# cebarker1000/heatflow

Measured on AMD Instinct MI355X. Metric: DOF-updates/s (timesteps/s x nDOF) on geballe_with_diamond, higher is better.
Workload: dtype f64

## Files before the change

heatflow_amd/csrc/heatflow_hip.hip:

```cpp

#include "hf_amg_io.hpp"

namespace {

struct MeshTables {
  std::vector<int32_t> rowptr, colidx;
  ColDict spmv;
  RowGather rg;
  std::vector<char> tag_used;
  int max_blk_nnz = 0;
};

constexpr char BLOB_MAGIC[8] = {'H', 'F', 'P', 'A', 'T', '0', '2', 0};
struct BlobHeader {
  char magic[8];
  int64_t total_bytes, nnz;
  int32_t n, ne, rba, ts, max_blk_nnz, tab_len, rg_ok, rg_max_dict, spmv_max_dict, reserved;
  int64_t count[12];
};

void steady_swap(hf_ctx* ctx) {
  hf_ctx::Steady& S = ctx->steady;
  std::swap(ctx->nbc, S.nbc); std::swap(ctx->d_bc_dofs, S.bc_dofs); std::swap(ctx->d_g, S.g);
  std::swap(ctx->nlift_rows, S.nlift_rows); std::swap(ctx->nlift, S.nlift);
  std::swap(ctx->d_lift_rows, S.lift_rows); std::swap(ctx->d_lift_ptr, S.lift_ptr); std::swap(ctx->d_lift_bc, S.lift_bc);
  std::swap(ctx->d_lift_slot, S.lift_slot); std::swap(ctx->d_lift_val, S.lift_val);
  std::swap(ctx->d_A, S.K); std::swap(ctx->d_dinv, S.dinv);
  std::swap(ctx->amg, S.amg); std::swap(ctx->d_coarse_inv, S.coarse_inv); std::swap(ctx->d_coarse_inv_f, S.coarse_inv_f);
  std::swap(ctx->coarse_n, S.coarse_n); std::swap(ctx->coarse_ld, S.coarse_ld); std::swap(ctx->amg_ready, S.amg_ready);
  std::swap(ctx->amg_fine_stale, S.amg_fine_stale); std::swap(ctx->amg_opc, S.amg_opc); std::swap(ctx->amg_setup_s, S.amg_setup_s);
  std::swap(ctx->amg_print, S.amg_print);
}
struct SteadyScope {
  hf_ctx* c;
  explicit SteadyScope(hf_ctx* ctx) : c(ctx) { steady_swap(c); }
  ~SteadyScope() { steady_swap(c); }
  SteadyScope(const SteadyScope&) = delete;
  SteadyScope& operator=(const SteadyScope&) = delete;
};

void steady_free(hf_ctx* ctx) {
  {
    SteadyScope sw(ctx);
    free_amg(ctx);
  }
  hf_ctx::Steady& S = ctx->steady;
  dev_free(&S.bc_dofs); dev_free(&S.g); dev_free(&S.lift_rows); dev_free(&S.lift_ptr); dev_free(&S.lift_bc);
  dev_free(&S.lift_slot); dev_free(&S.lift_val); dev_free(&S.K); dev_free(&S.dinv); dev_free(&S.Kfree);
  S.nbc = S.nlift_rows = S.nlift = 0;
  S.ready = false;
  S.pred_iters = 0;
}

void load_free(hf_ctx* ctx) {
  dev_free(&ctx->d_load);
  ctx->have_load = false;
}

void tangent_free(hf_ctx* ctx) {
  free_batch_state(ctx->tanb);
  dev_free(&ctx->tan.col); dev_free(&ctx->tan.F);
  ctx->tan = hf_ctx::Tangent();
}
// ... 17 lines not shown
  ctx->max_chunk_nnz_s = 0;
  for (int c = 0; c < ctx->nchunks_s; ++c)
    ctx->max_chunk_nnz_s = std::max(ctx->max_chunk_nnz_s, T.rowptr[std::min<int64_t>(n, (c + 1LL) * SRPC)] - T.rowptr[static_cast<size_t>(c) * SRPC]);
  ctx->max_cdict = T.spmv.max_dict;
  ctx->c16 = true;
  if (const char* e = std::getenv("HEATFLOW_SPMV_C16")) ctx->c16 = (e[0] != '0');
  if (static_cast<size_t>(ctx->max_chunk_nnz_s + ctx->max_cdict) * 8 > 64 * 1024) ctx->c16 = false;
  ctx->cdict_own = static_cast<int>(T.spmv.ptr.size()) == ctx->nchunks_s + 1;
  for (int c = 0; c < ctx->nchunks_s && ctx->cdict_own; ++c) {
    const int32_t r0 = c * SRPC, r1 = std::min<int32_t>(n, r0 + SRPC);
    const int32_t* lo = T.spmv.dict.data() + T.spmv.ptr[c];
    const int32_t* hi = T.spmv.dict.data() + T.spmv.ptr[c + 1];
    const int32_t* at = std::lower_bound(lo, hi, r0);
    ctx->cdict_own = hi - at >= r1 - r0 && at[0] == r0 && at[r1 - r0 - 1] == r1 - 1;
  }
  ctx->max_blk_nnz = T.max_blk_nnz;
  if (static_cast<size_t>((ctx->max_blk_nnz + 1) & ~1) * 16 + (RBA + 1) * 4 > 160 * 1024)
    return fail(ctx, HF_ERR_ARG, "row block holds %d nonzeros: LDS slab too large", ctx->max_blk_nnz);
  ctx->tab_len = static_cast<int>(T.tag_used.size());
  ctx->h_tag_used = T.tag_used;
  ctx->assembled = false; ctx->have_mat = false;
  ctx->h_tri.assign(tri, tri + 3 * static_cast<size_t>(ne));
  ctx->h_tag.assign(tag, tag + ne);
  ctx->owner_ready = false;
  ctx->ncolors = 0; ctx->elist_len = 0;
  dev_free(&ctx->d_blk_eptr); dev_free(&ctx->d_blk_cptr); dev_free(&ctx->d_blk_ent);

  std::vector<int4> elem(ne);
  for (int32_t e = 0; e < ne; ++e) elem[e] = make_int4(tri[3 * e], tri[3 * e + 1], tri[3 * e + 2], tag[e]);
  HF_TRY(dev_alloc(ctx, &ctx->d_zr, n));
// ... 442 lines not shown
  *out = ctx;
  return rc;
}

int hf_destroy(hf_ctx* ctx) {
  if (!ctx) return HF_ERR_ARG;
  (void)hipSetDevice(ctx->dev);
  if (ctx->stream) (void)hipStreamSynchronize(ctx->stream);
  dev_free(&ctx->d_zr); dev_free(&ctx->d_elem); dev_free(&ctx->d_kappa); dev_free(&ctx->d_rhoc);
  dev_free(&ctx->d_rowptr); dev_free(&ctx->d_colidx); dev_free(&ctx->d_cdict_ptr); dev_free(&ctx->d_cdict); dev_free(&ctx->d_cid); dev_free(&ctx->d_blk_eptr); dev_free(&ctx->d_blk_cptr); dev_free(&ctx->d_blk_ent); dev_free(&ctx->d_rg_hdr); dev_free(&ctx->d_rg_ell); dev_free(&ctx->d_rg_cid); dev_free(&ctx->d_rg_dict); dev_free(&ctx->d_rg_zrb); dev_free(&ctx->d_kappa_rg); dev_free(&ctx->d_rhoc_rg); dev_free(&ctx->d_M); dev_free(&ctx->d_A); dev_free(&ctx->d_dinv);
  dev_free(&ctx->d_bc_dofs); dev_free(&ctx->d_g); dev_free(&ctx->d_lift_rows); dev_free(&ctx->d_lift_ptr);
  dev_free(&ctx->d_lift_bc); dev_free(&ctx->d_lift_slot); dev_free(&ctx->d_lift_val);
  dev_free(&ctx->d_uprev); dev_free(&ctx->d_ustart);
  dev_free(&ctx->d_u); dev_free(&ctx->d_b); dev_free(&ctx->d_r); dev_free(&ctx->d_p); dev_free(&ctx->d_Ap);
  free_batch(ctx); free_batch_state(ctx->fluxb); free_batch_cols(ctx); free_amg(ctx); free_responses(ctx); proj_free(ctx); dev_free(&ctx->d_z); dev_free(&ctx->d_z2);
  steady_free(ctx); load_free(ctx); tangent_free(ctx);
  dev_free(&ctx->d_M1); dev_free(&ctx->d_dinv1); dev_free(&ctx->d_gz); dev_free(&ctx->d_gr); dev_free(&ctx->d_bz); dev_free(&ctx->d_br);
  dev_free(&ctx->d_tmp); dev_free(&ctx->d_part_pAp); dev_free(&ctx->d_part_rz); dev_free(&ctx->d_part_zz);
  dev_free(&ctx->d_part_bn); dev_free(&ctx->d_scal); dev_free(&ctx->d_samp_idx); dev_free(&ctx->d_samp); dev_free(&ctx->d_fsamp_idx);
  for (auto& e : ctx->prof_ev) (void)hipEventDestroy(e);
  if (ctx->h_scal) (void)hipHostFree(ctx->h_scal);
  if (ctx->h_mirror) (void)hipHostFree(ctx->h_mirror);
  if (ctx->ev0) (void)hipEventDestroy(ctx->ev0);
  if (ctx->ev1) (void)hipEventDestroy(ctx->ev1);
  if (ctx->stream) (void)hipStreamDestroy(ctx->stream);
  delete ctx;
  return HF_OK;
}

int hf_set_mesh(hf_ctx* ctx, int32_t n, int32_t ne, const double* zr, const int32_t* tri, const int32_t* tag) {
  if (!ctx) return HF_ERR_ARG;
// ... 138 lines not shown
  ctx->dt = ctx->scheme == HF_TIME_BDF2 ? 2.0 * dt / 3.0 : dt;
  ctx->mode = mode;
  HF_HIP(hipEventRecord(ctx->ev0, ctx->stream));
  HF_TRY(launch_assemble(ctx));
  if (ctx->nbc > 0) {
    if (ctx->nlift > 0)
      hipLaunchKernelGGL(k_take_lift, dim3((ctx->nlift + 255) / 256), dim3(256), 0, ctx->stream, ctx->nlift,
                         ctx->d_lift_slot, ctx->d_A, ctx->d_lift_val);
    hipLaunchKernelGGL(k_bc_rows, dim3((ctx->nbc + 255) / 256), dim3(256), 0, ctx->stream, ctx->nbc, ctx->d_bc_dofs,
                       ctx->d_rowptr, ctx->d_colidx, ctx->d_A);
  }
  hipLaunchKernelGGL(k_dinv, dim3((ctx->n + 255) / 256), dim3(256), 0, ctx->stream, ctx->n, ctx->d_rowptr,
                     ctx->d_colidx, ctx->d_A, ctx->d_dinv);
  HF_HIP(hipEventRecord(ctx->ev1, ctx->stream));
  HF_HIP(hipGetLastError());
  HF_HIP(hipStreamSynchronize(ctx->stream));
  float ms = 0.f;
  HF_HIP(hipEventElapsedTime(&ms, ctx->ev0, ctx->ev1));
  ctx->last_ms = ms;
  if (ctx->precond == 1) {
    OperatorPrint now;
    HF_TRY(operator_print(ctx, now));
    if (!(ctx->amg_ready && ctx->amg_reuse)) {
      HF_TRY(build_amg_auto(ctx));
      ctx->amg_print = std::move(now);
    } else {
      ctx->amg_fine_stale = !same_print(now, ctx->amg_print);
    }
  }
  if (ctx->precond == 1 && ctx->amg_ready) {
    ctx->amg[0].A.val = ctx->d_A;
// ... 492 lines not shown
  HF_HIP(copy_sync(ctx, S.bc_dofs, dofs, sizeof(int32_t) * n_s, hipMemcpyHostToDevice));
  HF_HIP(hipEventRecord(ctx->ev0, ctx->stream));
  HF_TRY(launch_assemble_rows<true>(ctx, ctx->d_kappa_rg, ctx->d_rhoc_rg, 1.0, nullptr, S.Kfree));
  HF_HIP(hipMemcpyAsync(S.K, S.Kfree, sizeof(double) * ctx->nnz, hipMemcpyDeviceToDevice, ctx->stream));
  {
    SteadyScope sw(ctx);
    HF_TRY(build_lift(ctx));
    if (ctx->nlift > 0)
      hipLaunchKernelGGL(k_take_lift, dim3((ctx->nlift + 255) / 256), dim3(256), 0, ctx->stream, ctx->nlift, ctx->d_lift_slot,
                         ctx->d_A, ctx->d_lift_val);
    hipLaunchKernelGGL(k_bc_rows, dim3((ctx->nbc + 255) / 256), dim3(256), 0, ctx->stream, ctx->nbc, ctx->d_bc_dofs, ctx->d_rowptr,
                       ctx->d_colidx, ctx->d_A);
    hipLaunchKernelGGL(k_dinv, dim3((n + 255) / 256), dim3(256), 0, ctx->stream, n, ctx->d_rowptr, ctx->d_colidx, ctx->d_A, ctx->d_dinv);
    HF_HIP(hipEventRecord(ctx->ev1, ctx->stream));
    HF_HIP(hipGetLastError());
    HF_HIP(hipStreamSynchronize(ctx->stream));
    float ms = 0.f;
    HF_HIP(hipEventElapsedTime(&ms, ctx->ev0, ctx->ev1));
    ctx->last_ms = ms;
    if (precond == 1) HF_TRY(build_amg_auto(ctx));
  }
  S.precond = precond;
  S.pred_iters = 0;
  S.ready = true;
  return HF_OK;
}

int hf_steady_solve(hf_ctx* ctx, const double* g_s, int32_t use_load, double rtol, double atol, int32_t max_it, int32_t* iters,
                    double* resid) {
  if (!ctx) return HF_ERR_ARG;
  if (!ctx->steady.ready) return fail(ctx, HF_ERR_STATE, "hf_steady_solve before hf_steady_setup (or the materials changed since)");
// ... 433 lines not shown
```

heatflow_amd/csrc/hf_context.hpp:

```cpp

#pragma once
#include <hip/hip_runtime.h>
#include <hip/hip_ext.h>

#include <algorithm>
#include <chrono>
#include <cmath>
#include <cstdarg>
#include <cstdint>
#include <cstdio>
#include <cstdlib>
#include <cstring>
#include <string>
#include <thread>
#include <vector>

#include "amg_host.hpp"
#include "heatflow_hip.h"

namespace {

constexpr int RB = 256;
#ifndef HF_RBA
#define HF_RBA 256
// ... 60 lines not shown
  hipStream_t stream = nullptr;
  hipEvent_t ev0 = nullptr, ev1 = nullptr;
  std::string err;
  double last_ms = 0.0;

  int32_t n = 0, ne = 0, nbc = 0;
  int64_t nnz = 0;
  int nchunks = 0, P = 0;
  int nchunks_s = 0, Ps = 0;
  int max_chunk_nnz_s = 0;
  int32_t *d_cdict_ptr = nullptr, *d_cdict = nullptr;
  uint16_t* d_cid = nullptr;
  int max_cdict = 0;
  bool cdict_own = false;
  bool c16 = true;
  bool have_mesh = false, have_mat = false, assembled = false;
  double dt = 0.0;
  double dt_step = 0.0;
  int mode = 0;
  int scheme = HF_TIME_BACKWARD_EULER;

  std::vector<int32_t> h_rowptr, h_colidx, h_tri, h_tag;
  std::vector<char> h_tag_used;
  bool owner_ready = false;

  double2* d_zr = nullptr;
  int4* d_elem = nullptr;
  int tab_len = 0;
  double *d_kappa = nullptr, *d_rhoc = nullptr;
  int32_t *d_rowptr = nullptr, *d_colidx = nullptr;
// ... 64 lines not shown
    double *dinv = nullptr, *x = nullptr, *cat = nullptr, *b = nullptr, *res = nullptr;
    bool own_b = false;
    double omega = 0; int n = 0;
  };
  std::vector<DevLevel> amg;
  double* d_coarse_inv = nullptr;
  float* d_coarse_inv_f = nullptr;
  int coarse_n = 0, coarse_ld = 0;
  bool amg_fine_stale = false;
  int amg_fuse0 = 0;
  bool amg_f32 = true;
  double amg_opc = 0.0, amg_setup_s = 0.0;
  struct OperatorPrint { double dt = 0.0; std::vector<double> kappa, rhoc; int32_t nbc = 0; uint64_t bc_hash = 0; int32_t scheme = 0; } amg_print;
  long long amg_fallbacks = 0;
  struct Steady {
    bool ready = false;
    int precond = 0, pred_iters = 0;
    int32_t nbc = 0, nlift_rows = 0, nlift = 0;
    int32_t *bc_dofs = nullptr, *lift_rows = nullptr, *lift_ptr = nullptr, *lift_bc = nullptr, *lift_slot = nullptr;
    double *g = nullptr, *lift_val = nullptr, *K = nullptr, *dinv = nullptr, *Kfree = nullptr;
    std::vector<DevLevel> amg;
    double* coarse_inv = nullptr;
    float* coarse_inv_f = nullptr;
    int coarse_n = 0, coarse_ld = 0;
    bool amg_ready = false, amg_fine_stale = false;
    double amg_opc = 0.0, amg_setup_s = 0.0;
    OperatorPrint amg_print;
  } steady;
  double* d_load = nullptr;
  bool have_load = false;
// ... 121 lines not shown
```

heatflow_amd/csrc/hf_kernels.hpp:

```cpp
#pragma once
#include "hf_context.hpp"

namespace {


template <int NW = 4>
__device__ __forceinline__ double block_sum(double v, double* sw) {
#pragma unroll
  for (int o = 32; o > 0; o >>= 1) v += __shfl_down(v, o, 64);
  const int w = threadIdx.x >> 6;
  if ((threadIdx.x & 63) == 0) sw[w] = v;
  __syncthreads();
  double t = sw[0];
#pragma unroll
  for (int k = 1; k < NW; ++k) t += sw[k];
  __syncthreads();
  return t;
}

__device__ __forceinline__ double sum_partials(const double* __restrict__ part, int P, double* s4) {
  double v = 0.0;
  for (int k = threadIdx.x; k < P; k += TPB) v += part[k];
  return block_sum(v, s4);
}
// ... 507 lines not shown
  const int q = blockIdx.x * blockDim.x + threadIdx.x;
  if (q < ns) out[q] = u[idx[q]];
}

__global__ __launch_bounds__(TPB) void k_hold_load(int n, const int32_t* __restrict__ rowptr, const int32_t* __restrict__ colidx,
                                                   const double* __restrict__ K, const double* __restrict__ u,
                                                   const unsigned char* __restrict__ mask, double* __restrict__ F) {
  const int row = blockIdx.x * blockDim.x + threadIdx.x;
  if (row >= n) return;
  double s = 0.0;
  if (!mask[row])
    for (int k = rowptr[row]; k < rowptr[row + 1]; ++k) s += K[k] * u[colidx[k]];
  F[row] = s;
}

__global__ void k_mark_rows(int nq, const int32_t* __restrict__ idx, unsigned char* __restrict__ mask) {
  const int q = blockIdx.x * blockDim.x + threadIdx.x;
  if (q < nq) mask[idx[q]] = 1;
}

__device__ __forceinline__ unsigned long long mirror_stamp(unsigned epoch, int v) {
  return (static_cast<unsigned long long>(epoch) << 32) | static_cast<unsigned>(v);
}
__device__ __forceinline__ void mirror_publish(ScalMirror* m, double zz, int iters, int done, unsigned epoch) {
  if (m == nullptr) return;
  m->zz = zz;
  m->iters = iters;
  __hip_atomic_store(&m->done_st, mirror_stamp(epoch, done), __ATOMIC_RELAXED, __HIP_MEMORY_SCOPE_SYSTEM);
  __threadfence_system();
  __hip_atomic_store(&m->tested_st, mirror_stamp(epoch, iters + 1), __ATOMIC_RELEASE, __HIP_MEMORY_SCOPE_SYSTEM);
}
__device__ __forceinline__ void mirror_breakdown(ScalMirror* m, unsigned epoch) {
  if (m != nullptr) __hip_atomic_store(&m->done_st, mirror_stamp(epoch, 2), __ATOMIC_RELEASE, __HIP_MEMORY_SCOPE_SYSTEM);
}

struct ColComp { const int32_t* dptr; const int32_t* dict; const uint16_t* id; int xd_off; int own; };

#ifndef HF_NT_STREAM
#define HF_NT_STREAM 0
#endif
#ifndef HF_PIPE
#define HF_PIPE 1
#endif
#ifndef HF_PHASE_CLOCK
#define HF_PHASE_CLOCK -1
#endif
#if HF_PHASE_CLOCK >= 0
#ifndef HF_PHASE_CONV
#define HF_PHASE_CONV 0
#endif
__device__ unsigned long long g_phase[MAXP * 16];
// ... 2 lines not shown
    if (MODE == HF_PHASE_CLOCK && C16 && (MODE != 0 || (part2 != nullptr) == (HF_PHASE_CONV != 0)) && threadIdx.x == 0 && (slot) < 16) \
      g_phase[blockIdx.x * 16 + (slot)] = wall_clock64();                                                \
  } while (0)
#else
#define HF_STAMP(slot) do { } while (0)
#endif
template <typename T>
__device__ __forceinline__ T stream_load(const T* p) {
#if HF_NT_STREAM
  return __builtin_nontemporal_load(p);
#else
  return *p;
#endif
}

__device__ __forceinline__ double bdf2_operand(double un, double unm1) { return (4.0 * un - unm1) * (1.0 / 3.0); }

template <int MODE, bool C16 = false, typename VT = double, int UN = 8>
__global__ __launch_bounds__(TS) __attribute__((amdgpu_waves_per_eu(8, 8))) void k_spmv(int n, int nchunks, int rpc ,
                                              const int32_t* __restrict__ rowptr, const int32_t* __restrict__ colidx,
                                              const VT* __restrict__ vals, const double* __restrict__ x,
                                              double* __restrict__ y, Scal* __restrict__ scal,
                                              double* __restrict__ part0, const double* __restrict__ bvec,
                                              const double* __restrict__ dinv, double* __restrict__ pvec,
                                              double* __restrict__ part1, double* __restrict__ part2, double w,
                                              int npart ,
                                              int parity, ColComp comp) {
  extern __shared__ double sprod[];
  __shared__ double s4[TS / 64];
  __shared__ int s_own;
  constexpr bool BDF = MODE >= 12 && MODE <= 15;
  auto opnd = [&](int c) { return BDF ? bdf2_operand(x[c], bvec[c]) : x[c]; };
  if ((MODE == 3 || MODE == 4 || MODE == 6 || MODE == 9) && scal->done) return;
  if ((MODE == 0 || MODE == 7) && scal != nullptr && scal->done) return;
  double acc0 = 0.0, acc1 = 0.0, acc2 = 0.0;
  double beta = 0.0;
  bool first9 = false;
  if (MODE == 9) {
    first9 = scal->first != 0;
    if (!first9) {
      double v0 = 0.0, v1 = 0.0, v2 = 0.0;
      for (int k = threadIdx.x; k < npart; k += TS) {
        v0 += part1[parity * MAXP + k];
        v1 += part1[(parity ^ 1) * MAXP + k];
        v2 += part2[k];
// ... 10 lines not shown
      beta = rz_new / rz_old;
    }
  }
  auto cycle_gate = [&]() {
    if (!((MODE == 3 || MODE == 0) && part2 != nullptr)) return false;
    double v2 = 0.0;
    for (int k = threadIdx.x; k < npart; k += TS) v2 += part2[k];
    const double zz = block_sum<TS / 64>(v2, s4);
    const bool conv = zz <= scal->tol2;
    if (blockIdx.x == 0 && threadIdx.x == 0) {
      if (conv) { scal->zz = zz; scal->done = 1; }
      mirror_publish(scal->mirror, zz, scal->iters, conv ? 1 : 0, scal->epoch);
    }
    return conv;
  };
  constexpr bool PIPELINED = C16 && (HF_PIPE == 2 || (HF_PIPE == 1 && sizeof(VT) == 4));
  if (!PIPELINED && cycle_gate()) return;
  const ChunkIter sched(nchunks);
  HF_STAMP(0);
  int stamp_at = 1;
  (void)stamp_at;
  const int tpr = (MODE == 0 || MODE == 6 || MODE == 7) ? TS / rpc : 1;
  const int prel = static_cast<int>(threadIdx.x) / tpr;
  const int psub = static_cast<int>(threadIdx.x) % tpr;
  struct RowOps { double b, d, y, p, x; };
  auto row_operands = [&](int prc, bool from_slice) {
    RowOps e{0.0, 0.0, 0.0, 0.0, 0.0};
    if (MODE == 2 || MODE == 3 || MODE == 4 || MODE == 5 || MODE == 7 || MODE == 8 || MODE == 11 || MODE == 13 || MODE == 15) e.b = bvec[prc];
    if (MODE == 2 || MODE == 4 || MODE == 5 || MODE == 10 || MODE == 11 || MODE == 14 || MODE == 15) e.d = dinv[prc];
    if (MODE == 6 || (MODE == 9 && !first9)) e.y = y[prc];
    if (MODE == 9 && !first9) e.p = pvec[prc];
    if ((MODE == 4 || MODE == 8 || MODE == 9 || MODE == 11) && !from_slice) e.x = x[prc];
    if (BDF) e.x = x[prc];
    return e;
  };
  auto rows_phase = [&](bool pin, int prow, int pa, int pb, const RowOps& e) {
    if ((MODE == 0 || MODE == 6 || MODE == 7) && tpr > 1) {
      double s = 0.0;
      if (pin)
        for (int j = pa + psub; j < pb; j += tpr) s += sprod[j];
      for (int o = tpr >> 1; o > 0; o >>= 1) s += __shfl_down(s, o, 64);
      if (pin && psub == 0) {
        y[prow] = (MODE == 6) ? e.y + s : s;
        if (MODE == 7) acc0 += e.b * s;
      }
    } else if (pin) {
      const int row = prow;
      double s = 0.0;
      for (int j = pa; j < pb; ++j) s += sprod[j];
      if (MODE == 0) {
        y[row] = s;
      } else if (MODE == 2) {
        const double ri = e.b - s;
        const double zi = e.d * ri;
        y[row] = ri;
        pvec[row] = zi;
        acc0 += ri * zi;
        acc1 += zi * zi;
        acc2 += (e.d * e.b) * (e.d * e.b);
      } else if (MODE == 3) {
        y[row] = e.b - s;
      } else if (MODE == 4) {
        const double yi = e.x + w * e.d * (e.b - s);
        y[row] = yi;
// ... 125 lines not shown
    }
  } else {
  const ChunkIter& sched_ = sched;
  for (int chunk = sched_.chunk; chunk < sched_.end; chunk += sched_.step) {
    const int r0 = chunk * rpc;
    const int r1 = min(n, r0 + rpc);
    const int k0 = rowptr[r0];
    const int k1 = rowptr[r1];
    const int prow = r0 + prel;
    const bool pin = prow < r1;
    int pa = 0, pb = 0;
    if (pin) {
      pa = rowptr[prow] - k0;
      pb = rowptr[prow + 1] - k0;
    }
    RowOps e = row_operands(min(prow, r1 - 1), C16 && comp.own != 0);
    if (C16) {
      double* xd = sprod + comp.xd_off;
      const int d0 = comp.dptr[chunk], nd = comp.dptr[chunk + 1] - d0;
      int k = k0 + threadIdx.x;
      double v[HF_UNROLL];
      int id[HF_UNROLL];
#pragma unroll
      for (int u = 0; u < HF_UNROLL; ++u) {
        const bool in = k + u * TS < k1;
        v[u] = in ? static_cast<double>(stream_load(&vals[k + u * TS])) : 0.0;
        id[u] = in ? static_cast<int>(stream_load(&comp.id[k + u * TS])) : 0;
      }
      for (int i = threadIdx.x; i < nd; i += HF_STAGE_U * TS) {
        int c[HF_STAGE_U];
        double xv[HF_STAGE_U];
#pragma unroll
        for (int u = 0; u < HF_STAGE_U; ++u) c[u] = (i + u * TS < nd) ? comp.dict[d0 + i + u * TS] : 0;
#pragma unroll
        for (int u = 0; u < HF_STAGE_U; ++u) xv[u] = (i + u * TS < nd) ? opnd(c[u]) : 0.0;
#pragma unroll
        for (int u = 0; u < HF_STAGE_U; ++u)
          if (i + u * TS < nd) {
            xd[i + u * TS] = xv[u];
            if ((MODE == 4 || MODE == 8 || MODE == 9 || MODE == 11) && c[u] == r0) s_own = i + u * TS;
          }
      }
      __syncthreads();
      HF_STAMP(stamp_at); ++stamp_at;
      if ((MODE == 4 || MODE == 8 || MODE == 9 || MODE == 11) && comp.own && pin) e.x = xd[s_own + (prow - r0)];
      while (k < k1) {
        const int kn = k + HF_UNROLL * TS;
        double vn[HF_UNROLL];
        int idn[HF_UNROLL];
#pragma unroll
        for (int u = 0; u < HF_UNROLL; ++u) {
          const bool in = kn + u * TS < k1;
          vn[u] = in ? static_cast<double>(stream_load(&vals[kn + u * TS])) : 0.0;
          idn[u] = in ? static_cast<int>(stream_load(&comp.id[kn + u * TS])) : 0;
        }
#pragma unroll
        for (int u = 0; u < HF_UNROLL; ++u)
          if (k + u * TS < k1) sprod[k - k0 + u * TS] = v[u] * xd[id[u]];
#pragma unroll
        for (int u = 0; u < HF_UNROLL; ++u) { v[u] = vn[u]; id[u] = idn[u]; }
        k = kn;
      }
    } else {
      for (int k = k0 + threadIdx.x; k < k1; k += HF_UNROLL * TS) {
        int c[HF_UNROLL];
        double v[HF_UNROLL], xv[HF_UNROLL];
#pragma unroll
        for (int u = 0; u < HF_UNROLL; ++u) {
          const bool in = k + u * TS < k1;
          c[u] = in ? colidx[k + u * TS] : 0;
          v[u] = in ? static_cast<double>(vals[k + u * TS]) : 0.0;
        }
#pragma unroll
        for (int u = 0; u < HF_UNROLL; ++u) xv[u] = (k + u * TS < k1) ? opnd(c[u]) : 0.0;
#pragma unroll
        for (int u = 0; u < HF_UNROLL; ++u)
          if (k + u * TS < k1) sprod[k - k0 + u * TS] = v[u] * xv[u];
      }
    }
    __syncthreads();
    HF_STAMP(stamp_at); ++stamp_at;
    rows_phase(pin, prow, pa, pb, e);
    __syncthreads();
    HF_STAMP(stamp_at); ++stamp_at;
  }
  }
  if (MODE == 2 || MODE == 7 || MODE == 9 || (MODE == 4 && part0 != nullptr)) {
    const double t0 = block_sum<TS / 64>(acc0, s4);
    if (threadIdx.x == 0) {
      part0[blockIdx.x] = t0;
      for (int q = blockIdx.x + gridDim.x; q < npart; q += gridDim.x) part0[q] = 0.0;
    }
  }
  if (MODE == 2 || MODE == 5) {
    const double t1 = block_sum<TS / 64>(acc1, s4);
    const double t2 = block_sum<TS / 64>(acc2, s4);
    if (threadIdx.x == 0) {
// ... 534 lines not shown
```

heatflow_amd/csrc/hf_pattern.hpp:

```cpp
#pragma once
#include <thread>

#include "hf_kernels.hpp"

namespace {

struct ColDict {
  std::vector<int32_t> ptr, dict;
  std::vector<uint16_t> id;
  int max_dict = 0;
};

struct RowGather {
  bool ok = false;
  std::vector<int4> hdr;
  std::vector<uint16_t> ell;
  std::vector<int32_t> tags;
  ColDict cols;
};

struct OwnerLists {
  std::vector<int32_t> blk_eptr, blk_cptr, blk_elist;
  std::vector<int2> blk_ent;
  int ncolors = 0;
// ... 331 lines not shown
  if (ctx->mode == HF_ASM_ROW_GATHER)
    return launch_assemble_lds(ctx, true, ctx->d_kappa, ctx->d_rhoc, ctx->dt, ctx->d_M, ctx->d_A);
  if (ctx->mode == HF_ASM_LDS_COLORED || ctx->mode == HF_ASM_LDS_ATOMIC) {
    return launch_assemble_lds(ctx, ctx->mode == HF_ASM_LDS_COLORED, ctx->d_kappa, ctx->d_rhoc, ctx->dt, ctx->d_M, ctx->d_A);
  } else {
    HF_HIP(hipMemsetAsync(ctx->d_M, 0, sizeof(double) * ctx->nnz, ctx->stream));
    HF_HIP(hipMemsetAsync(ctx->d_A, 0, sizeof(double) * ctx->nnz, ctx->stream));
    hipLaunchKernelGGL(k_assemble_global, dim3((ctx->ne + TPB - 1) / TPB), dim3(TPB), 0, ctx->stream, ctx->ne,
                       ctx->d_rowptr, ctx->d_colidx, ctx->d_elem, ctx->d_zr, ctx->d_kappa, ctx->d_rhoc, ctx->dt,
                       ctx->d_M, ctx->d_A);
  }
  HF_HIP(hipGetLastError());
  return HF_OK;
}

template <int MODE, typename VT = double>
void launch_spmv(hf_ctx* c, const VT* vals, const double* x, double* y, double* part0 = nullptr,
                 const double* bvec = nullptr, double* pvec = nullptr, double* part1 = nullptr,
                 double* part2 = nullptr, double w = 0.0, const double* dinv = nullptr, hipEvent_t ev_start = nullptr,
                 hipEvent_t ev_stop = nullptr, int parity = 0) {
  const ColComp comp{c->d_cdict_ptr, c->d_cdict, c->d_cid, c->max_chunk_nnz_s, c->cdict_own ? 1 : 0};
#define HF_SPMV_ARGS c->n, c->nchunks_s, static_cast<int>(SRPC), static_cast<const int32_t*>(c->d_rowptr),                    \
                     static_cast<const int32_t*>(c->d_colidx), vals, x, y, (MODE == 0 ? nullptr : c->d_scal), part0, bvec,  \
                     dinv ? dinv : static_cast<const double*>(c->d_dinv), pvec, part1, part2, w, c->P, parity, comp
  const std::uint32_t smem = static_cast<std::uint32_t>(spmv_smem_bytes(c));
  if (c->c16) {
    if (ev_start != nullptr) hipExtLaunchKernelGGL((k_spmv<MODE, true, VT, HF_SPMV_UN>), dim3(c->Ps), dim3(TS), smem, c->stream, ev_start, ev_stop, 0u, HF_SPMV_ARGS);
    else hipLaunchKernelGGL((k_spmv<MODE, true, VT, HF_SPMV_UN>), dim3(c->Ps), dim3(TS), smem, c->stream, HF_SPMV_ARGS);
  } else {
    if (ev_start != nullptr) hipExtLaunchKernelGGL((k_spmv<MODE, false, VT>), dim3(c->Ps), dim3(TS), smem, c->stream, ev_start, ev_stop, 0u, HF_SPMV_ARGS);
    else hipLaunchKernelGGL((k_spmv<MODE, false, VT>), dim3(c->Ps), dim3(TS), smem, c->stream, HF_SPMV_ARGS);
  }
#undef HF_SPMV_ARGS
}

constexpr int PROF_PAIRS = 64;

struct LinSys { const double* A; const double* dinv; double* x; const double* b; };

void launch_pcg_iteration(hf_ctx* c, const LinSys& s, int parity) {
// ... 11 lines not shown
```

Baseline: 730.9 million.

## Stream half-stored symmetric matrix values in SpMV to cut value traffic

```diff
diff --git a/heatflow_amd/csrc/heatflow_hip.hip b/heatflow_amd/csrc/heatflow_hip.hip
--- a/heatflow_amd/csrc/heatflow_hip.hip
+++ b/heatflow_amd/csrc/heatflow_hip.hip
@@ -25,7 +25,7 @@
   std::swap(ctx->nlift_rows, S.nlift_rows); std::swap(ctx->nlift, S.nlift);
   std::swap(ctx->d_lift_rows, S.lift_rows); std::swap(ctx->d_lift_ptr, S.lift_ptr); std::swap(ctx->d_lift_bc, S.lift_bc);
   std::swap(ctx->d_lift_slot, S.lift_slot); std::swap(ctx->d_lift_val, S.lift_val);
-  std::swap(ctx->d_A, S.K); std::swap(ctx->d_dinv, S.dinv);
+  std::swap(ctx->d_A, S.K); std::swap(ctx->d_dinv, S.dinv); std::swap(ctx->sym_A, S.symK);
   std::swap(ctx->amg, S.amg); std::swap(ctx->d_coarse_inv, S.coarse_inv); std::swap(ctx->d_coarse_inv_f, S.coarse_inv_f);
   std::swap(ctx->coarse_n, S.coarse_n); std::swap(ctx->coarse_ld, S.coarse_ld); std::swap(ctx->amg_ready, S.amg_ready);
   std::swap(ctx->amg_fine_stale, S.amg_fine_stale); std::swap(ctx->amg_opc, S.amg_opc); std::swap(ctx->amg_setup_s, S.amg_setup_s);
@@ -47,6 +47,7 @@
   hf_ctx::Steady& S = ctx->steady;
   dev_free(&S.bc_dofs); dev_free(&S.g); dev_free(&S.lift_rows); dev_free(&S.lift_ptr); dev_free(&S.lift_bc);
   dev_free(&S.lift_slot); dev_free(&S.lift_val); dev_free(&S.K); dev_free(&S.dinv); dev_free(&S.Kfree);
+  sym_free_vals(S.symK);
   S.nbc = S.nlift_rows = S.nlift = 0;
   S.ready = false;
   S.pred_iters = 0;
@@ -94,6 +95,9 @@
     const int32_t* at = std::lower_bound(lo, hi, r0);
     ctx->cdict_own = hi - at >= r1 - r0 && at[0] == r0 && at[r1 - r0 - 1] == r1 - 1;
   }
+  ctx->sym = true;
+  if (const char* e = std::getenv("HEATFLOW_SPMV_SYM")) ctx->sym = (e[0] != '0');
+  HF_TRY(sym_install_layout(ctx, T.rowptr, T.colidx, T.spmv.id));
   ctx->max_blk_nnz = T.max_blk_nnz;
   if (static_cast<size_t>((ctx->max_blk_nnz + 1) & ~1) * 16 + (RBA + 1) * 4 > 160 * 1024)
     return fail(ctx, HF_ERR_ARG, "row block holds %d nonzeros: LDS slab too large", ctx->max_blk_nnz);
@@ -566,7 +570,7 @@
   dev_free(&ctx->d_uprev); dev_free(&ctx->d_ustart);
   dev_free(&ctx->d_u); dev_free(&ctx->d_b); dev_free(&ctx->d_r); dev_free(&ctx->d_p); dev_free(&ctx->d_Ap);
   free_batch(ctx); free_batch_state(ctx->fluxb); free_batch_cols(ctx); free_amg(ctx); free_responses(ctx); proj_free(ctx); dev_free(&ctx->d_z); dev_free(&ctx->d_z2);
-  steady_free(ctx); load_free(ctx); tangent_free(ctx);
+  steady_free(ctx); load_free(ctx); tangent_free(ctx); sym_free_layout(ctx);
   dev_free(&ctx->d_M1); dev_free(&ctx->d_dinv1); dev_free(&ctx->d_gz); dev_free(&ctx->d_gr); dev_free(&ctx->d_bz); dev_free(&ctx->d_br);
   dev_free(&ctx->d_tmp); dev_free(&ctx->d_part_pAp); dev_free(&ctx->d_part_rz); dev_free(&ctx->d_part_zz);
   dev_free(&ctx->d_part_bn); dev_free(&ctx->d_scal); dev_free(&ctx->d_samp_idx); dev_free(&ctx->d_samp); dev_free(&ctx->d_fsamp_idx);
@@ -735,7 +739,11 @@
                      ctx->d_colidx, ctx->d_A, ctx->d_dinv);
   HF_HIP(hipEventRecord(ctx->ev1, ctx->stream));
   HF_HIP(hipGetLastError());
-  HF_HIP(hipStreamSynchronize(ctx->stream));
+  HF_TRY(sym_debug_flip(ctx));
+  HF_TRY(sym_gather(ctx, ctx->sym_A, ctx->d_A, 0));
+  HF_TRY(sym_gather(ctx, ctx->sym_M, ctx->d_M, 1));
+  HF_HIP(hipStreamSynchronize(ctx->stream));
+  HF_TRY(sym_check(ctx, &ctx->sym_A, &ctx->sym_M));
   float ms = 0.f;
   HF_HIP(hipEventElapsedTime(&ms, ctx->ev0, ctx->ev1));
   ctx->last_ms = ms;
@@ -1258,7 +1266,9 @@
     hipLaunchKernelGGL(k_dinv, dim3((n + 255) / 256), dim3(256), 0, ctx->stream, n, ctx->d_rowptr, ctx->d_colidx, ctx->d_A, ctx->d_dinv);
     HF_HIP(hipEventRecord(ctx->ev1, ctx->stream));
     HF_HIP(hipGetLastError());
+    HF_TRY(sym_gather(ctx, ctx->sym_A, ctx->d_A, 0));
     HF_HIP(hipStreamSynchronize(ctx->stream));
+    HF_TRY(sym_check(ctx, &ctx->sym_A, nullptr));
     float ms = 0.f;
     HF_HIP(hipEventElapsedTime(&ms, ctx->ev0, ctx->ev1));
     ctx->last_ms = ms;
diff --git a/heatflow_amd/csrc/hf_context.hpp b/heatflow_amd/csrc/hf_context.hpp
--- a/heatflow_amd/csrc/hf_context.hpp
+++ b/heatflow_amd/csrc/hf_context.hpp
@@ -98,6 +98,19 @@
   int max_cdict = 0;
   bool cdict_own = false;
   bool c16 = true;
+  bool sym = true;
+  bool sym_layout = false;
+  int64_t sym_nl = 0, sym_ns = 0;
+  int32_t *d_sym_lptr = nullptr, *d_sym_lsrc = nullptr, *d_sym_pmap = nullptr, *d_sym_dsrc = nullptr, *d_sym_sptr = nullptr,
+          *d_sym_ssrc = nullptr;
+  uint32_t *d_sym_lw = nullptr, *d_sym_sw = nullptr;
+  int* d_sym_bad = nullptr;
+  struct SymVals {
+    const double* src = nullptr;
+    double *lval = nullptr, *dval = nullptr, *sval = nullptr;
+    bool ok = false;
+  };
+  SymVals sym_A, sym_M;
   bool have_mesh = false, have_mat = false, assembled = false;
   double dt = 0.0;
   double dt_step = 0.0;
@@ -192,6 +205,7 @@
   struct OperatorPrint { double dt = 0.0; std::vector<double> kappa, rhoc; int32_t nbc = 0; uint64_t bc_hash = 0; int32_t scheme = 0; } amg_print;
   long long amg_fallbacks = 0;
   struct Steady {
+    SymVals symK;
     bool ready = false;
     int precond = 0, pred_iters = 0;
     int32_t nbc = 0, nlift_rows = 0, nlift = 0;
diff --git a/heatflow_amd/csrc/hf_kernels.hpp b/heatflow_amd/csrc/hf_kernels.hpp
--- a/heatflow_amd/csrc/hf_kernels.hpp
+++ b/heatflow_amd/csrc/hf_kernels.hpp
@@ -545,6 +545,24 @@
   F[row] = s;
 }
 
+__global__ __launch_bounds__(TPB) void k_sym_gather(int64_t nl, int n, int64_t ns, const int32_t* __restrict__ lsrc,
+                                                    const int32_t* __restrict__ pmap, const int32_t* __restrict__ dsrc,
+                                                    const int32_t* __restrict__ ssrc, const double* __restrict__ vals,
+                                                    double* __restrict__ lval, double* __restrict__ dval,
+                                                    double* __restrict__ sval, int* __restrict__ bad) {
+  const int64_t q = static_cast<int64_t>(blockIdx.x) * blockDim.x + threadIdx.x;
+  if (q < nl) {
+    const double v = vals[lsrc[q]];
+    lval[q] = v;
+    const int32_t kp = pmap[q];
+    if (kp >= 0 && __double_as_longlong(vals[kp]) != __double_as_longlong(v)) *bad = 1;
+  } else if (q < nl + n) {
+    dval[q - nl] = vals[dsrc[q - nl]];
+  } else if (q < nl + n + ns) {
+    sval[q - nl - n] = vals[ssrc[q - nl - n]];
+  }
+}
+
 __global__ void k_mark_rows(int nq, const int32_t* __restrict__ idx, unsigned char* __restrict__ mask) {
   const int q = blockIdx.x * blockDim.x + threadIdx.x;
   if (q < nq) mask[idx[q]] = 1;
@@ -565,7 +583,11 @@
   if (m != nullptr) __hip_atomic_store(&m->done_st, mirror_stamp(epoch, 2), __ATOMIC_RELEASE, __HIP_MEMORY_SCOPE_SYSTEM);
 }
 
-struct ColComp { const int32_t* dptr; const int32_t* dict; const uint16_t* id; int xd_off; int own; };
+struct ColComp {
+  const int32_t* dptr; const int32_t* dict; const uint16_t* id; int xd_off; int own;
+  const int32_t* lptr = nullptr; const double* lval = nullptr; const uint32_t* lw = nullptr; const double* dval = nullptr;
+  const int32_t* sptr = nullptr; const double* sval = nullptr; const uint32_t* sw = nullptr;
+};
 
 #ifndef HF_NT_STREAM
 #define HF_NT_STREAM 0
@@ -598,9 +620,14 @@
 #endif
 }
 
+__device__ __forceinline__ double add_rounded_product(double s, double a, double b) {
+#pragma clang fp contract(off)
+  return s + a * b;
+}
+
 __device__ __forceinline__ double bdf2_operand(double un, double unm1) { return (4.0 * un - unm1) * (1.0 / 3.0); }
 
-template <int MODE, bool C16 = false, typename VT = double, int UN = 8>
+template <int MODE, bool C16 = false, typename VT = double, int UN = 8, bool SYM = false>
 __global__ __launch_bounds__(TS) __attribute__((amdgpu_waves_per_eu(8, 8))) void k_spmv(int n, int nchunks, int rpc ,
                                               const int32_t* __restrict__ rowptr, const int32_t* __restrict__ colidx,
                                               const VT* __restrict__ vals, const double* __restrict__ x,
@@ -610,9 +637,11 @@
                                               double* __restrict__ part1, double* __restrict__ part2, double w,
                                               int npart ,
                                               int parity, ColComp comp) {
+  static_assert(!SYM || (C16 && sizeof(VT) == 8 && MODE != 6 && MODE != 7), "half-stored stream: fine-level double operators");
   extern __shared__ double sprod[];
   __shared__ double s4[TS / 64];
   __shared__ int s_own;
+  constexpr bool OWNX = SYM || MODE == 4 || MODE == 8 || MODE == 9 || MODE == 11;
   constexpr bool BDF = MODE >= 12 && MODE <= 15;
   auto opnd = [&](int c) { return BDF ? bdf2_operand(x[c], bvec[c]) : x[c]; };
   if ((MODE == 3 || MODE == 4 || MODE == 6 || MODE == 9) && scal->done) return;
@@ -653,7 +682,7 @@
     }
     return conv;
   };
-  constexpr bool PIPELINED = C16 && (HF_PIPE == 2 || (HF_PIPE == 1 && sizeof(VT) == 4));
+  constexpr bool PIPELINED = C16 && !SYM && (HF_PIPE == 2 || (HF_PIPE == 1 && sizeof(VT) == 4));
   if (!PIPELINED && cycle_gate()) return;
   const ChunkIter sched(nchunks);
   HF_STAMP(0);
@@ -662,22 +691,28 @@
   const int tpr = (MODE == 0 || MODE == 6 || MODE == 7) ? TS / rpc : 1;
   const int prel = static_cast<int>(threadIdx.x) / tpr;
   const int psub = static_cast<int>(threadIdx.x) % tpr;
-  struct RowOps { double b, d, y, p, x; };
+  struct RowOps { double b, d, y, p, x, dg; };
   auto row_operands = [&](int prc, bool from_slice) {
-    RowOps e{0.0, 0.0, 0.0, 0.0, 0.0};
+    RowOps e{0.0, 0.0, 0.0, 0.0, 0.0, 0.0};
     if (MODE == 2 || MODE == 3 || MODE == 4 || MODE == 5 || MODE == 7 || MODE == 8 || MODE == 11 || MODE == 13 || MODE == 15) e.b = bvec[prc];
     if (MODE == 2 || MODE == 4 || MODE == 5 || MODE == 10 || MODE == 11 || MODE == 14 || MODE == 15) e.d = dinv[prc];
     if (MODE == 6 || (MODE == 9 && !first9)) e.y = y[prc];
     if (MODE == 9 && !first9) e.p = pvec[prc];
     if ((MODE == 4 || MODE == 8 || MODE == 9 || MODE == 11) && !from_slice) e.x = x[prc];
     if (BDF) e.x = x[prc];
+    if (SYM) e.dg = comp.dval[prc];
     return e;
   };
-  auto rows_phase = [&](bool pin, int prow, int pa, int pb, const RowOps& e) {
+  auto rows_phase = [&](bool pin, int prow, int pa, int pb, const RowOps& e, double xi = 0.0, int ua = 0, int ub = 0) {
     if ((MODE == 0 || MODE == 6 || MODE == 7) && tpr > 1) {
       double s = 0.0;
-      if (pin)
+      if (pin && SYM) {
+        const int nl = pb - pa, len = nl + 1 + (ub - ua);
+        for (int q = psub; q < len; q += tpr)
+          s = q < nl ? s + sprod[pa + q] : (q == nl ? add_rounded_product(s, e.dg, xi) : s + sprod[ua + q - nl - 1]);
+      } else if (pin) {
         for (int j = pa + psub; j < pb; j += tpr) s += sprod[j];
+      }
       for (int o = tpr >> 1; o > 0; o >>= 1) s += __shfl_down(s, o, 64);
       if (pin && psub == 0) {
         y[prow] = (MODE == 6) ? e.y + s : s;
@@ -687,6 +722,10 @@
       const int row = prow;
       double s = 0.0;
       for (int j = pa; j < pb; ++j) s += sprod[j];
+      if (SYM) {
+        s = add_rounded_product(s, e.dg, xi);
+        for (int j = ua; j < ub; ++j) s += sprod[j];
+      }
       if (MODE == 0) {
         y[row] = s;
       } else if (MODE == 2) {
@@ -842,18 +881,47 @@
       pa = rowptr[prow] - k0;
       pb = rowptr[prow + 1] - k0;
     }
+    int l0 = 0, l1 = 0, ua = 0, ub = 0, s0 = 0, s1 = 0;
+    if (SYM) {
+      l0 = comp.lptr[r0];
+      l1 = comp.lptr[r1];
+      s0 = comp.sptr[chunk];
+      s1 = comp.sptr[chunk + 1];
+      if (pin) {
+        const int la = comp.lptr[prow] - l0, lb = comp.lptr[prow + 1] - l0, nlc = l1 - l0;
+        ua = nlc + pa - la - (prow - r0);
+        ub = nlc + pb - lb - (prow - r0) - 1;
+        pa = la;
+        pb = lb;
+      }
+    }
     RowOps e = row_operands(min(prow, r1 - 1), C16 && comp.own != 0);
     if (C16) {
       double* xd = sprod + comp.xd_off;
       const int d0 = comp.dptr[chunk], nd = comp.dptr[chunk + 1] - d0;
-      int k = k0 + threadIdx.x;
+      const int kend = SYM ? l1 : k1;
+      const int klast = max(kend - 1, 0);
+      int k = (SYM ? l0 : k0) + threadIdx.x;
       double v[HF_UNROLL];
       int id[HF_UNROLL];
 #pragma unroll
       for (int u = 0; u < HF_UNROLL; ++u) {
-        const bool in = k + u * TS < k1;
-        v[u] = in ? static_cast<double>(stream_load(&vals[k + u * TS])) : 0.0;
-        id[u] = in ? static_cast<int>(stream_load(&comp.id[k + u * TS])) : 0;
+        if (SYM) {
+          const int kk = min(k + u * TS, klast);
+          v[u] = stream_load(&comp.lval[kk]);
+          id[u] = static_cast<int>(stream_load(&comp.lw[kk]));
+        } else {
+          const bool in = k + u * TS < k1;
+          v[u] = in ? static_cast<double>(stream_load(&vals[k + u * TS])) : 0.0;
+          id[u] = in ? static_cast<int>(stream_load(&comp.id[k + u * TS])) : 0;
+        }
+      }
+      double sv = 0.0;
+      unsigned sw = 0;
+      if (SYM) {
+        const int q = min(s0 + static_cast<int>(threadIdx.x), max(s1 - 1, 0));
+        sv = stream_load(&comp.sval[q]);
+        sw = stream_load(&comp.sw[q]);
       }
       for (int i = threadIdx.x; i < nd; i += HF_STAGE_U * TS) {
         int c[HF_STAGE_U];
@@ -866,28 +934,53 @@
         for (int u = 0; u < HF_STAGE_U; ++u)
           if (i + u * TS < nd) {
             xd[i + u * TS] = xv[u];
-            if ((MODE == 4 || MODE == 8 || MODE == 9 || MODE == 11) && c[u] == r0) s_own = i + u * TS;
+            if (OWNX && c[u] == r0) s_own = i + u * TS;
           }
       }
       __syncthreads();
       HF_STAMP(stamp_at); ++stamp_at;
       if ((MODE == 4 || MODE == 8 || MODE == 9 || MODE == 11) && comp.own && pin) e.x = xd[s_own + (prow - r0)];
-      while (k < k1) {
+      const int own = SYM ? s_own : 0;
+      while (k < kend) {
         const int kn = k + HF_UNROLL * TS;
         double vn[HF_UNROLL];
         int idn[HF_UNROLL];
 #pragma unroll
         for (int u = 0; u < HF_UNROLL; ++u) {
-          const bool in = kn + u * TS < k1;
-          vn[u] = in ? static_cast<double>(stream_load(&vals[kn + u * TS])) : 0.0;
-          idn[u] = in ? static_cast<int>(stream_load(&comp.id[kn + u * TS])) : 0;
+          if (SYM) {
+            const int kk = min(kn + u * TS, klast);
+            vn[u] = stream_load(&comp.lval[kk]);
+            idn[u] = static_cast<int>(stream_load(&comp.lw[kk]));
+          } else {
+            const bool in = kn + u * TS < k1;
+            vn[u] = in ? static_cast<double>(stream_load(&vals[kn + u * TS])) : 0.0;
+            idn[u] = in ? static_cast<int>(stream_load(&comp.id[kn + u * TS])) : 0;
+          }
         }
 #pragma unroll
         for (int u = 0; u < HF_UNROLL; ++u)
-          if (k + u * TS < k1) sprod[k - k0 + u * TS] = v[u] * xd[id[u]];
+          if (k + u * TS < kend) {
+            if (SYM) {
+              const unsigned w = static_cast<unsigned>(id[u]), slot = w >> 21;
+              sprod[k - l0 + u * TS] = v[u] * xd[w & 0xFFFu];
+              if (slot != 0x7FFu) sprod[(l1 - l0) + slot] = v[u] * xd[own + ((w >> 12) & 0x1FFu)];
+            } else {
+              sprod[k - k0 + u * TS] = v[u] * xd[id[u]];
+            }
+          }
 #pragma unroll
         for (int u = 0; u < HF_UNROLL; ++u) { v[u] = vn[u]; id[u] = idn[u]; }
         k = kn;
+      }
+      if (SYM) {
+        for (int qb = s0;;) {
+          if (qb + static_cast<int>(threadIdx.x) < s1) sprod[(l1 - l0) + (sw >> 16)] = sv * xd[sw & 0xFFFFu];
+          qb += TS;
+          if (qb >= s1) break;
+          const int q = min(qb + static_cast<int>(threadIdx.x), s1 - 1);
+          sv = stream_load(&comp.sval[q]);
+          sw = stream_load(&comp.sw[q]);
+        }
       }
     } else {
       for (int k = k0 + threadIdx.x; k < k1; k += HF_UNROLL * TS) {
@@ -908,7 +1001,8 @@
     }
     __syncthreads();
     HF_STAMP(stamp_at); ++stamp_at;
-    rows_phase(pin, prow, pa, pb, e);
+    if (SYM) rows_phase(pin, prow, pa, pb, e, pin ? sprod[comp.xd_off + s_own + (prow - r0)] : 0.0, ua, ub);
+    else rows_phase(pin, prow, pa, pb, e);
     __syncthreads();
     HF_STAMP(stamp_at); ++stamp_at;
   }
diff --git a/heatflow_amd/csrc/hf_pattern.hpp b/heatflow_amd/csrc/hf_pattern.hpp
--- a/heatflow_amd/csrc/hf_pattern.hpp
+++ b/heatflow_amd/csrc/hf_pattern.hpp
@@ -1,7 +1,9 @@
 #pragma once
 #include <thread>
+#include <type_traits>
 
 #include "hf_kernels.hpp"
+#include "hf_sym_layout.hpp"
 
 namespace {
 
@@ -369,6 +371,89 @@
   return HF_OK;
 }
 
+void sym_free_vals(hf_ctx::SymVals& s) {
+  dev_free(&s.lval); dev_free(&s.dval); dev_free(&s.sval);
+  s.src = nullptr; s.ok = false;
+}
+void sym_free_layout(hf_ctx* ctx) {
+  dev_free(&ctx->d_sym_lptr); dev_free(&ctx->d_sym_lsrc); dev_free(&ctx->d_sym_pmap); dev_free(&ctx->d_sym_dsrc);
+  dev_free(&ctx->d_sym_sptr); dev_free(&ctx->d_sym_ssrc); dev_free(&ctx->d_sym_lw); dev_free(&ctx->d_sym_sw); dev_free(&ctx->d_sym_bad);
+  sym_free_vals(ctx->sym_A); sym_free_vals(ctx->sym_M); sym_free_vals(ctx->steady.symK);
+  ctx->sym_layout = false; ctx->sym_nl = ctx->sym_ns = 0;
+}
+int sym_install_layout(hf_ctx* ctx, const std::vector<int32_t>& rowptr, const std::vector<int32_t>& colidx,
+                       const std::vector<uint16_t>& cid) {
+  sym_free_layout(ctx);
+  if (!ctx->sym || !ctx->c16 || !ctx->cdict_own || SRPC > TS) return HF_OK;
+  SymLayout L;
+  if (!build_sym_layout(rowptr, colidx, cid, ctx->n, SRPC, L, host_threads())) {
+    if (std::getenv("HEATFLOW_DEBUG")) std::fprintf(stderr, "[set_mesh] half-stored stream not used: %s\n", L.why.c_str());
+    return HF_OK;
+  }
+  ctx->sym_nl = static_cast<int64_t>(L.lsrc.size());
+  ctx->sym_ns = static_cast<int64_t>(L.ssrc.size());
+  HF_TRY(dev_alloc(ctx, &ctx->d_sym_lptr, L.lptr.size()));
+  HF_TRY(dev_alloc(ctx, &ctx->d_sym_lsrc, L.lsrc.size()));
+  HF_TRY(dev_alloc(ctx, &ctx->d_sym_pmap, L.pmap.size()));
+  HF_TRY(dev_alloc(ctx, &ctx->d_sym_lw, L.lw.size()));
+  HF_TRY(dev_alloc(ctx, &ctx->d_sym_dsrc, L.dsrc.size()));
+  HF_TRY(dev_alloc(ctx, &ctx->d_sym_sptr, L.sptr.size()));
+  HF_TRY(dev_alloc(ctx, &ctx->d_sym_ssrc, L.ssrc.size()));
+  HF_TRY(dev_alloc(ctx, &ctx->d_sym_sw, L.sw.size()));
+  HF_TRY(dev_alloc(ctx, &ctx->d_sym_bad, 2));
+  auto up = [&](auto* d, const auto& h) { return h.empty() ? hipSuccess : copy_sync(ctx, d, h.data(), sizeof(h[0]) * h.size(), hipMemcpyHostToDevice); };
+  HF_HIP(up(ctx->d_sym_lptr, L.lptr)); HF_HIP(up(ctx->d_sym_lsrc, L.lsrc)); HF_HIP(up(ctx->d_sym_pmap, L.pmap));
+  HF_HIP(up(ctx->d_sym_lw, L.lw)); HF_HIP(up(ctx->d_sym_dsrc, L.dsrc)); HF_HIP(up(ctx->d_sym_sptr, L.sptr));
+  HF_HIP(up(ctx->d_sym_ssrc, L.ssrc)); HF_HIP(up(ctx->d_sym_sw, L.sw));
+  ctx->sym_layout = true;
+  return HF_OK;
+}
+int sym_gather(hf_ctx* ctx, hf_ctx::SymVals& s, const double* vals, int slot) {
+  s.ok = false;
+  s.src = nullptr;
+  if (!ctx->sym_layout) return HF_OK;
+  if (s.lval == nullptr) {
+    HF_TRY(dev_alloc(ctx, &s.lval, ctx->sym_nl));
+    HF_TRY(dev_alloc(ctx, &s.dval, ctx->n));
+    HF_TRY(dev_alloc(ctx, &s.sval, ctx->sym_ns));
+  }
+  HF_HIP(hipMemsetAsync(ctx->d_sym_bad + slot, 0, sizeof(int), ctx->stream));
+  const int64_t total = ctx->sym_nl + ctx->n + ctx->sym_ns;
+  hipLaunchKernelGGL(k_sym_gather, dim3(static_cast<unsigned>((total + TPB - 1) / TPB)), dim3(TPB), 0, ctx->stream, ctx->sym_nl,
+                     ctx->n, ctx->sym_ns, ctx->d_sym_lsrc, ctx->d_sym_pmap, ctx->d_sym_dsrc, ctx->d_sym_ssrc, vals, s.lval, s.dval,
+                     s.sval, ctx->d_sym_bad + slot);
+  HF_HIP(hipGetLastError());
+  s.src = vals;
+  return HF_OK;
+}
+int sym_debug_flip(hf_ctx* ctx) {
+  static const bool on = [] { const char* e = std::getenv("HEATFLOW_DEBUG_SYM_FLIP"); return e != nullptr && e[0] == '1'; }();
+  if (!on) return HF_OK;
+  for (int32_t i = ctx->n / 2; i < ctx->n; ++i)
+    for (int32_t k = ctx->h_rowptr[i]; k < ctx->h_rowptr[i + 1]; ++k) {
+      const int32_t j = ctx->h_colidx[k];
+      if (j <= i || j / SRPC != i / SRPC) continue;
+      uint64_t bits = 0;
+      HF_HIP(copy_sync(ctx, &bits, ctx->d_A + k, sizeof(bits), hipMemcpyDeviceToHost));
+      bits ^= uint64_t(1) << 30;
+      HF_HIP(copy_sync(ctx, ctx->d_A + k, &bits, sizeof(bits), hipMemcpyHostToDevice));
+      return HF_OK;
+    }
+  return HF_OK;
+}
+
+int sym_check(hf_ctx* ctx, hf_ctx::SymVals* a, hf_ctx::SymVals* b) {
+  if (!ctx->sym_layout) return HF_OK;
+  int bad[2] = {1, 1};
+  HF_HIP(copy_sync(ctx, bad, ctx->d_sym_bad, sizeof(bad), hipMemcpyDeviceToHost));
+  if (a != nullptr) a->ok = a->src != nullptr && bad[0] == 0;
+  if (b != nullptr) b->ok = b->src != nullptr && bad[1] == 0;
+  if (std::getenv("HEATFLOW_DEBUG"))
+    std::fprintf(stderr, "[sym] operator %s, mass %s\n", a == nullptr ? "-" : (a->ok ? "half-stored" : "full stream"),
+                 b == nullptr ? "-" : (b->ok ? "half-stored" : "full stream"));
+  return HF_OK;
+}
+
 template <int MODE, typename VT = double>
 void launch_spmv(hf_ctx* c, const VT* vals, const double* x, double* y, double* part0 = nullptr,
                  const double* bvec = nullptr, double* pvec = nullptr, double* part1 = nullptr,
@@ -379,6 +464,25 @@
                      static_cast<const int32_t*>(c->d_colidx), vals, x, y, (MODE == 0 ? nullptr : c->d_scal), part0, bvec,  \
                      dinv ? dinv : static_cast<const double*>(c->d_dinv), pvec, part1, part2, w, c->P, parity, comp
   const std::uint32_t smem = static_cast<std::uint32_t>(spmv_smem_bytes(c));
+  if constexpr (std::is_same<VT, double>::value) {
+    const hf_ctx::SymVals* sv = nullptr;
+    if (c->sym_layout && c->c16 && vals != nullptr) {
+      if (c->sym_A.ok && vals == c->sym_A.src) sv = &c->sym_A;
+      else if (c->sym_M.ok && vals == c->sym_M.src) sv = &c->sym_M;
+    }
+    if (sv != nullptr) {
+      ColComp sc = comp;
+      sc.lptr = c->d_sym_lptr; sc.lval = sv->lval; sc.lw = c->d_sym_lw; sc.dval = sv->dval;
+      sc.sptr = c->d_sym_sptr; sc.sval = sv->sval; sc.sw = c->d_sym_sw;
+#define HF_SPMV_SARGS c->n, c->nchunks_s, static_cast<int>(SRPC), static_cast<const int32_t*>(c->d_rowptr),                  \
+                      static_cast<const int32_t*>(c->d_colidx), vals, x, y, (MODE == 0 ? nullptr : c->d_scal), part0, bvec, \
+                      dinv ? dinv : static_cast<const double*>(c->d_dinv), pvec, part1, part2, w, c->P, parity, sc
+      if (ev_start != nullptr) hipExtLaunchKernelGGL((k_spmv<MODE, true, double, HF_SPMV_UN, true>), dim3(c->Ps), dim3(TS), smem, c->stream, ev_start, ev_stop, 0u, HF_SPMV_SARGS);
+      else hipLaunchKernelGGL((k_spmv<MODE, true, double, HF_SPMV_UN, true>), dim3(c->Ps), dim3(TS), smem, c->stream, HF_SPMV_SARGS);
+#undef HF_SPMV_SARGS
+      return;
+    }
+  }
   if (c->c16) {
     if (ev_start != nullptr) hipExtLaunchKernelGGL((k_spmv<MODE, true, VT, HF_SPMV_UN>), dim3(c->Ps), dim3(TS), smem, c->stream, ev_start, ev_stop, 0u, HF_SPMV_ARGS);
     else hipLaunchKernelGGL((k_spmv<MODE, true, VT, HF_SPMV_UN>), dim3(c->Ps), dim3(TS), smem, c->stream, HF_SPMV_ARGS);
diff --git a/heatflow_amd/csrc/hf_sym_layout.hpp b/heatflow_amd/csrc/hf_sym_layout.hpp
--- /dev/null
+++ b/heatflow_amd/csrc/hf_sym_layout.hpp
@@ -0,0 +1,118 @@
+#pragma once
+#include <algorithm>
+#include <cstdint>
+#include <string>
+#include <thread>
+#include <vector>
+
+struct SymLayout {
+  static constexpr uint32_t NO_SLOT = 0x7FF;
+  static constexpr int MAX_ID = 4096, MAX_ROWS = 512, MAX_SLOTS = 0x7FF;
+  bool ok = false;
+  std::string why;
+  std::vector<int32_t> lptr;
+  std::vector<int32_t> lsrc, pmap;
+  std::vector<uint32_t> lw;
+  std::vector<int32_t> dsrc;
+  std::vector<int32_t> sptr;
+  std::vector<int32_t> ssrc;
+  std::vector<uint32_t> sw;
+  int64_t n_pairs_in_chunk = 0;
+};
+
+inline bool build_sym_layout(const std::vector<int32_t>& rowptr, const std::vector<int32_t>& colidx,
+                             const std::vector<uint16_t>& cid, int32_t n, int rows, SymLayout& L, int threads = 1) {
+  L = SymLayout();
+  auto refuse = [&](const std::string& why) { L.ok = false; L.why = why; return false; };
+  if (rows <= 0 || rows > SymLayout::MAX_ROWS) return refuse("rows per chunk outside the 9-bit row field");
+  if (static_cast<int64_t>(rowptr.size()) != n + 1LL || cid.size() != colidx.size()) return refuse("inconsistent pattern");
+  const int nchunk = (n + rows - 1) / rows;
+  L.lptr.assign(static_cast<size_t>(n) + 1, 0);
+  L.dsrc.assign(n, -1);
+  L.sptr.assign(static_cast<size_t>(nchunk) + 1, 0);
+  auto find = [&](int32_t row, int32_t col) -> int64_t {
+    const int32_t* b = colidx.data() + rowptr[row];
+    const int32_t* e = colidx.data() + rowptr[row + 1];
+    const int32_t* at = std::lower_bound(b, e, col);
+    return (at != e && *at == col) ? at - colidx.data() : -1;
+  };
+  std::vector<std::string> err(nchunk);
+  auto over_chunks = [&](auto&& body) {
+    const int nt = std::max(1, std::min(threads, nchunk));
+    std::vector<std::thread> th;
+    for (int t = 1; t < nt; ++t)
+      th.emplace_back([&, t]() { for (int c = static_cast<int>(int64_t(nchunk) * t / nt); c < int64_t(nchunk) * (t + 1) / nt; ++c) body(c); });
+    for (int c = 0; c < int64_t(nchunk) / nt; ++c) body(c);
+    for (auto& x : th) x.join();
+    for (int c = 0; c < nchunk; ++c)
+      if (!err[c].empty()) return refuse(err[c]);
+    return true;
+  };
+  if (!over_chunks([&](int c) {
+        const int32_t r0 = c * rows, r1 = std::min<int32_t>(n, r0 + rows);
+        int32_t nup = 0, nspill = 0;
+        for (int32_t i = r0; i < r1 && err[c].empty(); ++i) {
+          int32_t nl = 0;
+          for (int64_t k = rowptr[i]; k < rowptr[i + 1]; ++k) {
+            const int32_t j = colidx[k];
+            if (j == i) { L.dsrc[i] = static_cast<int32_t>(k); continue; }
+            if (find(j, i) < 0) { err[c] = "pattern not structurally symmetric"; break; }
+            if (j < i) {
+              ++nl;
+              if (cid[k] >= SymLayout::MAX_ID) { err[c] = "column list longer than the 12-bit position field"; break; }
+            } else {
+              ++nup;
+              if (j >= r1) ++nspill;
+            }
+          }
+          if (L.dsrc[i] < 0 && err[c].empty()) err[c] = "row " + std::to_string(i) + " stores no diagonal";
+          L.lptr[i + 1] = nl;
+        }
+        if (nup > SymLayout::MAX_SLOTS && err[c].empty())
+          err[c] = "chunk " + std::to_string(c) + " holds more upper entries than the 11-bit slot field";
+        L.sptr[c + 1] = nspill;
+      }))
+    return false;
+  for (int32_t i = 0; i < n; ++i) L.lptr[i + 1] += L.lptr[i];
+  for (int c = 0; c < nchunk; ++c) L.sptr[c + 1] += L.sptr[c];
+  const int64_t nl_all = L.lptr[n];
+  L.lsrc.resize(nl_all);
+  L.lw.resize(nl_all);
+  L.pmap.resize(nl_all);
+  L.ssrc.resize(L.sptr[nchunk]);
+  L.sw.resize(L.sptr[nchunk]);
+  std::vector<int64_t> pairs(nchunk, 0);
+  over_chunks([&](int c) {
+    const int32_t r0 = c * rows, r1 = std::min<int32_t>(n, r0 + rows);
+    const int64_t k0 = rowptr[r0];
+    std::vector<int32_t> slot(static_cast<size_t>(rowptr[r1] - k0), -1);
+    int32_t ns = 0;
+    for (int32_t row = r0; row < r1; ++row)
+      for (int64_t k = rowptr[row]; k < rowptr[row + 1]; ++k)
+        if (colidx[k] > row) slot[k - k0] = ns++;
+    int64_t q = L.lptr[r0], s = L.sptr[c];
+    for (int32_t j = r0; j < r1; ++j)
+      for (int64_t k = rowptr[j]; k < rowptr[j + 1]; ++k) {
+        const int32_t i = colidx[k];
+        if (i > j) {
+          if (i >= r1) {
+            L.ssrc[s] = static_cast<int32_t>(k);
+            L.sw[s++] = static_cast<uint32_t>(cid[k]) | (static_cast<uint32_t>(slot[k - k0]) << 16);
+          }
+          continue;
+        }
+        if (i == j) continue;
+        const bool in = i >= r0;
+        const int64_t kp = in ? find(i, j) : -1;
+        L.lsrc[q] = static_cast<int32_t>(k);
+        L.pmap[q] = static_cast<int32_t>(kp);
+        L.lw[q] = static_cast<uint32_t>(cid[k]) | (static_cast<uint32_t>(j - r0) << 12) |
+                  ((in ? static_cast<uint32_t>(slot[kp - k0]) : SymLayout::NO_SLOT) << 21);
+        if (in) ++pairs[c];
+        ++q;
+      }
+  });
+  for (int c = 0; c < nchunk; ++c) L.n_pairs_in_chunk += pairs[c];
+  L.ok = true;
+  return true;
+}
```

New measurement: 747.9 million, median of 6. 1.02x the previous value.
